# scroll-tech/zkvm-prover

Measured on AMD Instinct MI355X. Metric: chunk STARK proofs/sec (2^22-row trace), higher is better.
Workload: dtype u32; 1 GPU; full STARK proof: 2^22 x 300 degree-3 AIR + 2^22 x 2 Fibonacci AIR, blow-up 2, 100 queries, PoW 16+16 (SURVEY.md 8(d) cfg #4); proof_bytes=1128348, resident_key_bytes_per_pipeline=13503716096, inflight_per_gpu=3, parallelism=3 independent proof(s) in flight per GPU (one HIP stream each)

## Files before the change

### include/zkhip.h

```cpp
#ifndef ZKHIP_H
#define ZKHIP_H
#include <stddef.h>
#include <stdint.h>

#ifdef __cplusplus
extern "C" {
#endif

#define ZKHIP_OK 0
#define ZKHIP_ERR_NO_DEVICE (-1)
#define ZKHIP_ERR_HIP (-2)
#define ZKHIP_ERR_INVALID (-3)
#define ZKHIP_ERR_NOMEM (-4)
#define ZKHIP_ERR_SMALL_BUFFER (-5)
#define ZKHIP_ERR_POW_FAILED (-6)
#define ZKHIP_ERR_VERIFY (-7)
#define ZKHIP_ERR_CONSTRAINT (-8)

#define ZKHIP_DIGEST_WORDS 8

typedef struct zkhip_ctx zkhip_ctx;

uint32_t zkhip_version(void);

// ... 455 lines not shown
int zkhip_recursion_air(const zkhip_recursion *r, size_t i, zkhip_air *out);
int zkhip_recursion_witness(zkhip_recursion *r, const uint8_t *const *proofs, const size_t *proof_lens, const uint32_t *const *const *child_pvs,
                            size_t n_present, uint32_t *node_pvs_out);
int zkhip_recursion_witness_uniform(zkhip_recursion *r, const uint8_t *const *proofs, const size_t *proof_lens, const uint32_t *const *const *child_pvs,
                                    const uint32_t *child_prep_commits, const int *child_is_leaf, const uint32_t leaf_commit[8],
                                    const uint32_t internal_commit[8], size_t n_present, uint32_t *node_pvs_out);
int zkhip_recursion_witness_deferral(zkhip_recursion *r, const uint8_t *const *proofs, const size_t *proof_lens, const uint32_t *const *const *child_pvs,
                                     const uint32_t *child_aux, const uint32_t acc_start[8], size_t n_present, uint32_t *node_pvs_out);
size_t zkhip_recursion_n_aux(const zkhip_recursion *r);
int zkhip_recursion_wires(const zkhip_recursion *r, uint32_t *out, size_t cap_words, size_t *n_words);
int zkhip_recursion_tracegen(zkhip_ctx *ctx, zkhip_recursion *r, uint32_t *d_gate_trace, uint32_t *d_p2_trace, uint32_t *d_pv_trace);

typedef struct {
    int host_sponge;
    uint32_t host_sponge_min_words;
    int jit;
    uint32_t jit_min_log_work;
    char jit_cache_dir[256];
    int quot_slices;
    uint32_t grind_sweep_shift;
    uint32_t coop_max_log, coop_inj_max_log;
    uint32_t top_max_log;
    uint32_t commit_parts, side_cus;
    uint32_t witness_threads;
    int pin_witness, parallel_queries;
    int self_check;
    int tree_store_early;
    uint32_t hash_block;
    int coop_fused;
    int rows_in_bulk;
    uint32_t rows_coop_max_log;
    uint32_t ntt_log_lanes;
    uint32_t quot_streams;
} zkhip_config;
int zkhip_tables_canonical(zkhip_ctx *ctx, int on);
int zkhip_jit_prewarm(const zkhip_air *airs, size_t n_airs, unsigned log_blowup, const char *cache_dir, size_t *n_ok);
void zkhip_config_default(zkhip_config *out);
unsigned zkhip_host_cpus(void);
int zkhip_ctx_get_config(zkhip_ctx *ctx, zkhip_config *out);
int zkhip_has_test_kernels(void);
int zkhip_ctx_set_config(zkhip_ctx *ctx, const zkhip_config *cfg);
int zkhip_set_process_config(const zkhip_config *cfg);

int zkhip_profile_enable(zkhip_ctx *ctx, int on);
typedef struct {
    char name[48];
    uint64_t launches;
    double total_ms;
} zkhip_kernel_stat;
int zkhip_profile_read(zkhip_ctx *ctx, zkhip_kernel_stat *out, size_t cap);
int zkhip_profile_reset(zkhip_ctx *ctx);

#ifdef __cplusplus
}
#endif
#endif
```

### integration/hip-backend/src/ffi.rs

```rust
#![allow(non_camel_case_types)]
use std::os::raw::{c_char, c_double, c_int, c_uint, c_void};

pub const ZKHIP_OK: c_int = 0;
pub const ZKHIP_ERR_NO_DEVICE: c_int = -1;
pub const ZKHIP_ERR_HIP: c_int = -2;
pub const ZKHIP_ERR_INVALID: c_int = -3;
pub const ZKHIP_ERR_NOMEM: c_int = -4;
pub const ZKHIP_ERR_SMALL_BUFFER: c_int = -5;
pub const ZKHIP_ERR_POW_FAILED: c_int = -6;
pub const ZKHIP_ERR_VERIFY: c_int = -7;
pub const ZKHIP_ERR_CONSTRAINT: c_int = -8;
pub const ZKHIP_DIGEST_WORDS: usize = 8;
pub const ZKHIP_KECCAK_F_WIDTH: usize = 2633;
pub const ZKHIP_INT256_ALU_WIDTH: usize = 101;
pub const ZKHIP_INT256_MUL_WIDTH: usize = 161;
pub const ZKHIP_MODMUL_WIDTH: usize = 325;
pub const ZKHIP_EC_WIDTH: usize = 772;
pub const ZKHIP_FP2_WIDTH: usize = 648;
pub const ZKHIP_FP2_RECORD_WORDS: usize = 33;
pub const ZKHIP_INT256_CMP_WIDTH: usize = 103;
pub const ZKHIP_INT256_SHIFT_WIDTH: usize = 189;
pub const ZKHIP_EC_RECORD_WORDS: usize = 41;
pub const ZKHIP_GKR_MAX_LOG_N: c_uint = 28;
pub const ZKHIP_WHIR_MAX_ROUNDS: usize = 32;
// ... 158 lines not shown
    pub uniform: c_int,
    pub min_log_height: [c_uint; 2],
    pub n_leaf_shapes: usize,
    pub app_id: *const u32,
    pub region_index: u32,
}

#[repr(C)]
#[derive(Clone, Copy)]
pub struct zkhip_config {
    pub host_sponge: c_int,
    pub host_sponge_min_words: u32,
    pub jit: c_int,
    pub jit_min_log_work: u32,
    pub jit_cache_dir: [c_char; 256],
    pub quot_slices: c_int,
    pub grind_sweep_shift: u32,
    pub coop_max_log: u32,
    pub coop_inj_max_log: u32,
    pub top_max_log: u32,
    pub commit_parts: u32,
    pub side_cus: u32,
    pub witness_threads: u32,
    pub pin_witness: c_int,
    pub parallel_queries: c_int,
    pub self_check: c_int,
    pub tree_store_early: c_int,
    pub hash_block: u32,
    pub coop_fused: c_int,
    pub rows_in_bulk: c_int,
    pub rows_coop_max_log: u32,
    pub ntt_log_lanes: u32,
    pub quot_streams: u32,
}

#[repr(C)]
#[derive(Clone, Copy)]
pub struct zkhip_kernel_stat {
    pub name: [c_char; 48],
    pub launches: u64,
    pub total_ms: c_double,
}

extern "C" {
    pub fn zkhip_version() -> u32;

    pub fn zkhip_ctx_create(device: c_int, out: *mut *mut zkhip_ctx) -> c_int;
    pub fn zkhip_ctx_destroy(ctx: *mut zkhip_ctx);
    pub fn zkhip_last_error(ctx: *const zkhip_ctx) -> *const c_char;
    pub fn zkhip_set_stream(ctx: *mut zkhip_ctx, hip_stream: *mut c_void) -> c_int;
    pub fn zkhip_sync(ctx: *mut zkhip_ctx) -> c_int;
    pub fn zkhip_set_commit_pipeline(ctx: *mut zkhip_ctx, parts: c_uint) -> c_int;
    pub fn zkhip_set_cu_partition(ctx: *mut zkhip_ctx, side_cus: c_uint) -> c_int;

    pub fn zkhip_malloc(ctx: *mut zkhip_ctx, bytes: usize, dptr: *mut *mut c_void) -> c_int;
    pub fn zkhip_free(ctx: *mut zkhip_ctx, dptr: *mut c_void) -> c_int;
    pub fn zkhip_h2d(ctx: *mut zkhip_ctx, dst: *mut c_void, src: *const c_void, bytes: usize) -> c_int;
    pub fn zkhip_d2h(ctx: *mut zkhip_ctx, dst: *mut c_void, src: *const c_void, bytes: usize) -> c_int;
    pub fn zkhip_host_alloc(ctx: *mut zkhip_ctx, bytes: usize, hptr: *mut *mut c_void) -> c_int;
    pub fn zkhip_host_free(ctx: *mut zkhip_ctx, hptr: *mut c_void) -> c_int;
    pub fn zkhip_h2d_async(ctx: *mut zkhip_ctx, dst: *mut c_void, src_pinned: *const c_void, bytes: usize) -> c_int;
    pub fn zkhip_zero(ctx: *mut zkhip_ctx, dptr: *mut c_void, bytes: usize) -> c_int;
    pub fn zkhip_to_monty(ctx: *mut zkhip_ctx, d: *mut u32, n: usize) -> c_int;
    pub fn zkhip_from_monty(ctx: *mut zkhip_ctx, d: *mut u32, n: usize) -> c_int;

    pub fn zkhip_ntt_batch(ctx: *mut zkhip_ctx, d_mat: *mut u32, log_n: c_uint, width: usize, stride: usize,
// ... 308 lines not shown
```

### zkvm-prover_amd/_binding.py

```python
import ctypes as C
import os
import re

import numpy as np

P = 2013265921
_HERE = os.path.dirname(os.path.abspath(__file__))
_ROOT = os.path.dirname(_HERE)
_LIB = None


class ZkhipError(RuntimeError):
    pass


def library_path():
    return os.path.join(_HERE, "libzkhip.so")


def declared_symbols():
    with open(os.path.join(_ROOT, "include", "zkhip.h")) as f:
        txt = f.read()
    txt = re.sub(r"/\*.*?\*/", "", txt, flags=re.S)
    return sorted(set(re.findall(r"\b(zkhip_[a-z0-9_]+)\s*\(", txt)))
# ... 24 lines not shown
        return p


class _Air(C.Structure):
    _fields_ = [("program", C.POINTER(C.c_uint32)), ("program_len", C.c_size_t), ("log_height", C.c_uint),
                ("width", C.c_size_t), ("n_pvs", C.c_size_t), ("prep_trace", C.POINTER(C.c_uint32)),
                ("prep_commit", C.POINTER(C.c_uint32))]


class _ProofLayout(C.Structure):
    _fields_ = [(n, C.c_size_t) for n in ("n_words", "root_main", "roots_cached", "n_cached", "root_perm", "exposed", "n_exposed", "root_quot", "opened",
                                          "n_opened", "fri_layers", "n_fri_layers", "final_poly", "n_final_poly", "query_pow", "queries",
                                          "query_words", "n_queries")]


class _V1Summary(C.Structure):
    _fields_ = [(n, C.c_size_t) for n in ("n_proofs", "n_airs", "n_queries", "n_fri_layers", "n_final_poly", "n_main_commits",
                                          "n_after_challenge_commits", "n_preprocessed", "n_input_batches")] + \
               [("log_max_height", C.c_uint), ("log_blowup", C.c_uint), ("has_logup_pow", C.c_int), ("log_degree", C.c_uint * 64)]


class _RecursionStmt(C.Structure):
    _fields_ = [("n_state", C.c_size_t), ("start_air", C.POINTER(C.c_uint32)), ("start_idx", C.POINTER(C.c_uint32)),
                ("end_air", C.POINTER(C.c_uint32)), ("end_idx", C.POINTER(C.c_uint32)), ("child_is_node", C.c_int),
                ("uniform", C.c_int), ("min_log_height", C.c_uint * 2), ("n_leaf_shapes", C.c_size_t), ("app_id", C.POINTER(C.c_uint32)),
                ("region_index", C.c_uint32)]


class Config(C.Structure):
    _fields_ = [("host_sponge", C.c_int), ("host_sponge_min_words", C.c_uint32), ("jit", C.c_int), ("jit_min_log_work", C.c_uint32),
                ("jit_cache_dir", C.c_char * 256), ("quot_slices", C.c_int), ("grind_sweep_shift", C.c_uint32), ("coop_max_log", C.c_uint32),
                ("coop_inj_max_log", C.c_uint32), ("top_max_log", C.c_uint32), ("commit_parts", C.c_uint32), ("side_cus", C.c_uint32), ("witness_threads", C.c_uint32),
                ("pin_witness", C.c_int), ("parallel_queries", C.c_int), ("self_check", C.c_int), ("tree_store_early", C.c_int), ("hash_block", C.c_uint32), ("coop_fused", C.c_int),
                ("rows_in_bulk", C.c_int), ("rows_coop_max_log", C.c_uint32), ("ntt_log_lanes", C.c_uint32), ("quot_streams", C.c_uint32)]

    @classmethod
    def default(cls):
        c = cls()
        load_library().zkhip_config_default(C.byref(c))
        return c


class _KernelStat(C.Structure):
    _fields_ = [("name", C.c_char * 48), ("launches", C.c_uint64), ("total_ms", C.c_double)]


def load_library():
    global _LIB
    if _LIB is not None:
        return _LIB
    path = library_path()
    if not os.path.exists(path):
        raise ZkhipError("libzkhip.so not built: run `python -c 'import __graft_entry__ as g; g.build()'` "
                         "(or make -C zkvm-prover_amd/csrc)")
    import torch

    lib = C.CDLL(path)
    vp, sz, u32p, uip = C.c_void_p, C.c_size_t, C.POINTER(C.c_uint32), C.POINTER(C.c_uint)
    sig = {
        "zkhip_version": (C.c_uint32, []),
        "zkhip_ctx_create": (C.c_int, [C.c_int, C.POINTER(vp)]),
        "zkhip_ctx_destroy": (None, [vp]),
        "zkhip_last_error": (C.c_char_p, [vp]),
        "zkhip_set_stream": (C.c_int, [vp, vp]),
        "zkhip_sync": (C.c_int, [vp]),
        "zkhip_set_commit_pipeline": (C.c_int, [vp, C.c_uint]),
        "zkhip_set_cu_partition": (C.c_int, [vp, C.c_uint]),
# ... 1616 lines not shown
```

### zkvm-prover_amd/csrc/api.hip

```cpp
#include <sched.h>
#include <cstring>
#include <thread>
#include <dlfcn.h>
#include <sys/stat.h>
#include <mutex>
#include <string.h>

#include <algorithm>
#include <mutex>
#include <unordered_map>

#include "transcript.hpp"
#include "zkhip_internal.hpp"

namespace zk {

int set_error(zkhip_ctx* ctx, int code, const std::string& msg) {
    if (ctx) ctx->last_error = msg;
    return code;
}

int get_scratch(zkhip_ctx* ctx, int slot, size_t bytes, void** out) {
    if (bytes == 0) bytes = 16;
    if (ctx->scratch_bytes[slot] < bytes) {
// ... 163 lines not shown
    }();
    return cached;
}

void zkhip_config_default(zkhip_config* c) {
    if (!c) return;
    auto num = [](const char* name, uint32_t dflt, uint32_t lo = 0, uint32_t hi = 0xffffffffu) {
        if (!getenv(name)) return dflt;
        const long long v = atoll(getenv(name));
        return (uint32_t)std::min<long long>(hi, std::max<long long>(lo, v));
    };
    memset(c, 0, sizeof *c);
    c->host_sponge = getenv("ZKHIP_NO_HOST_SPONGE") ? 0 : 1;
    c->host_sponge_min_words = num("ZKHIP_HOST_SPONGE_MIN_WORDS", 8192u);
    c->jit = getenv("ZKHIP_NO_JIT") ? 0 : getenv("ZKHIP_FORCE_JIT") ? 2 : 1;
    c->jit_min_log_work = num("ZKHIP_JIT_MIN_LOG_WORK", 26u, 0, 62);
    c->quot_slices = getenv("ZKHIP_NO_QUOT_SLICES") ? 0 : 1;
    c->grind_sweep_shift = num("ZKHIP_GRIND_SWEEP_SHIFT", 0u, 0, 8);
    c->coop_max_log = num("ZKHIP_COOP_MAX_LOG", 15u, 0, 27), c->coop_inj_max_log = num("ZKHIP_COOP_INJ_MAX_LOG", 15u, 0, 27);
    c->top_max_log = num("ZKHIP_TOP_MAX_LOG", 6u, 0, 8);
    c->commit_parts = num("ZKHIP_COMMIT_PARTS", 0u, 0, 8), c->side_cus = num("ZKHIP_SIDE_CUS", 0u);
    c->witness_threads = num("ZKHIP_WITNESS_THREADS", 0u);
    c->pin_witness = getenv("ZKHIP_NO_PIN_WITNESS") ? 0 : 1;
    c->parallel_queries = getenv("ZKHIP_RECURSION_SERIAL_QUERIES") ? 0 : 1;
    c->self_check = getenv("ZKHIP_SELF_CHECK") ? 1 : 0;
#ifdef ZKHIP_TEST_KERNELS
    c->tree_store_early = getenv("ZKHIP_TREE_STORE_EARLY") ? 1 : 0;
#endif
    c->hash_block = num("ZKHIP_HASH_BLOCK", 256u, 64, 768) / 64 * 64;
    c->coop_fused = getenv("ZKHIP_NO_COOP_FUSED") ? 0 : 1;
    c->rows_in_bulk = getenv("ZKHIP_NO_ROWS_IN_BULK") ? 0 : 1;
    c->rows_coop_max_log = num("ZKHIP_ROWS_COOP_MAX_LOG", 15u, 0, 27);
    c->ntt_log_lanes = num("ZKHIP_NTT_LOG_LANES", 10u, 8, 10);
    c->quot_streams = num("ZKHIP_QUOT_STREAMS", 0u, 0, 4);
    std::string dir;
    if (const char* e = getenv("ZKHIP_JIT_CACHE_DIR")) {
        dir = e;
    } else {
        Dl_info info;
        if (dladdr((const void*)&zkhip_config_default, &info) && info.dli_fname) {
            std::string p = info.dli_fname;
            const size_t slash = p.rfind('/');
            p = (slash == std::string::npos ? std::string(".") : p.substr(0, slash)) + "/jit_cache";
            struct stat st;
            if (stat(p.c_str(), &st) == 0 && S_ISDIR(st.st_mode)) dir = p;
        }
    }
    if (dir.size() < sizeof c->jit_cache_dir) memcpy(c->jit_cache_dir, dir.c_str(), dir.size() + 1);
}
extern "C++" {
namespace zk {
static zkhip_config g_process_config;
static std::once_flag g_process_config_once;
static std::mutex g_process_config_mu;
zkhip_config process_config() {
    std::call_once(g_process_config_once, [] { zkhip_config_default(&g_process_config); });
    std::lock_guard<std::mutex> lk(g_process_config_mu);
    return g_process_config;
}
}
}
int zkhip_set_process_config(const zkhip_config* cfg) {
    if (!cfg) return ZKHIP_ERR_INVALID;
    (void)zk::process_config();
    std::lock_guard<std::mutex> lk(zk::g_process_config_mu);
    zk::g_process_config = *cfg;
    return ZKHIP_OK;
}
int zkhip_tables_canonical(zkhip_ctx* ctx, int on) {
    if (!ctx) return ZKHIP_ERR_INVALID;
    ctx->tables_canonical = on != 0;
    return ZKHIP_OK;
}

int zkhip_has_test_kernels(void) {
#ifdef ZKHIP_TEST_KERNELS
    return 1;
#else
    return 0;
#endif
}

int zkhip_ctx_get_config(zkhip_ctx* ctx, zkhip_config* out) {
    if (!ctx || !out) return ZKHIP_ERR_INVALID;
    *out = ctx->cfg;
    return ZKHIP_OK;
}
int zkhip_ctx_set_config(zkhip_ctx* ctx, const zkhip_config* cfg) {
    if (!ctx || !cfg) return ZKHIP_ERR_INVALID;
    if (cfg->jit < 0 || cfg->jit > 2 || cfg->coop_max_log > 27 || cfg->coop_inj_max_log > 27 || cfg->rows_coop_max_log > 27 || cfg->ntt_log_lanes < 8 || cfg->ntt_log_lanes > 10 || cfg->quot_streams > 4 || cfg->jit_min_log_work > 62 || cfg->top_max_log > 8 || cfg->grind_sweep_shift > 8 ||
        cfg->commit_parts > 8 || cfg->side_cus >= (unsigned)ctx->cu_count || cfg->hash_block < 64 || cfg->hash_block > 768 || cfg->hash_block % 64)
        return set_error(ctx, ZKHIP_ERR_INVALID, "zkhip_ctx_set_config: field out of range (jit 0..2, coop_* <= 27, rows_coop_max_log <= 27, ntt_log_lanes 8..10, quot_streams <= 4, jit_min_log_work <= 62, top_max_log <= 8, grind_sweep_shift <= 8, commit_parts <= 8, side_cus < CUs, hash_block a multiple of 64 in 64..768)");
#ifndef ZKHIP_TEST_KERNELS
    if (cfg->tree_store_early)
        return set_error(ctx, ZKHIP_ERR_INVALID, "zkhip_ctx_set_config: tree_store_early names TEST kernels that this library was built without (libzkhip_test.so holds them)");
#endif
    ZK_TRY(zkhip_set_cu_partition(ctx, cfg->side_cus));
    ctx->cfg = *cfg;
    ctx->cfg.jit_cache_dir[sizeof ctx->cfg.jit_cache_dir - 1] = 0;
    ctx->commit_parts = cfg->commit_parts;
    return ZKHIP_OK;
}

void zkhip_ctx_destroy(zkhip_ctx* ctx) {
    if (!ctx) return;
    (void)hipSetDevice(ctx->device);
    (void)hipStreamSynchronize(ctx->stream);
    profile_flush(ctx);
    if (ctx->d_tw_fwd) (void)hipFree(ctx->d_tw_fwd);
    if (ctx->d_tw_inv) (void)hipFree(ctx->d_tw_inv);
    for (auto& kv : ctx->lde_tables) (void)hipFree(kv.second);
    for (int i = 0; i < 8; i++)
        if (ctx->scratch[i]) (void)hipFree(ctx->scratch[i]);
    if (ctx->side_stream) (void)hipStreamDestroy(ctx->side_stream);
    if (ctx->hash_stream) (void)hipStreamDestroy(ctx->hash_stream);
    for (auto& q : ctx->quot_streams)
        if (q) (void)hipStreamDestroy(q);
    if (ctx->quot_fork) (void)hipEventDestroy(ctx->quot_fork);
    for (auto& e : ctx->quot_join)
        if (e) (void)hipEventDestroy(e);
    if (ctx->d_deferred_bad) (void)hipFree(ctx->d_deferred_bad);
    if (ctx->gkr_ws) (void)hipFree(ctx->gkr_ws);
    if (ctx->h_sponge) (void)hipHostFree(ctx->h_sponge);
    if (ctx->own_stream) (void)hipStreamDestroy(ctx->own_stream);
    for (auto& e : ctx->pipe_ev)
// ... 340 lines not shown
```

### zkvm-prover_amd/csrc/ntt.hip

```cpp
#include <stdlib.h>
#include <string.h>

#include <algorithm>

#include "lds_barrier.hpp"
#include "zkhip_internal.hpp"

namespace zk {

__global__ void k_gen_twiddles(uint32_t* fwd, uint32_t* inv, uint32_t w, uint32_t winv, size_t half) {
    size_t e = (size_t)blockIdx.x * blockDim.x + threadIdx.x;
    if (e >= half) return;
    fwd[e] = mpow(w, e);
    inv[e] = mpow(winv, e);
}

int ensure_twiddles(zkhip_ctx* ctx, unsigned log_n) {
    if (log_n < 1) log_n = 1;
    if (log_n > 27) return set_error(ctx, ZKHIP_ERR_INVALID, "transform size exceeds two-adicity 27");
    if (ctx->tw_log >= log_n) return ZKHIP_OK;
    unsigned want = std::max(log_n, 16u);
    if (ctx->d_tw_fwd) {
        ZK_HIP_CHECK(ctx, hipStreamSynchronize(ctx->stream));
        ZK_HIP_CHECK(ctx, hipFree(ctx->d_tw_fwd));
// ... 403 lines not shown
#endif
        uint32_t* base = lv + j * pitch + c;
#pragma unroll
        for (int k = 0; k < 16; k++) base[(k << LOG_RQ) * pitch] = v[k];
    }
    zk_syncthreads();
#if !defined(NTT_ABL) || (NTT_ABL != 4 && NTT_ABL != 5)
    lds_rounds_ct<LOG_R, LOG_C, LOG_RQ, NT>(lv, twl, tid);
#endif
    const unsigned lo_mask = (1u << a.log_lo) - 1u;
    uint32_t* dst = (a.dst_cols ? a.dst_cols[mcol] : a.dst + mcol * a.dst_col_stride) + ((size_t)sub << a.log_m) + (size_t)X * a.out_x_stride;
    if constexpr (LOG_R >= LOG_T) {
        const uint32_t* lrow = lv + tid * pitch;
#pragma unroll
        for (unsigned i = 0; i < (R * C) / NT; i++) {
            const unsigned c = (NT * i) >> LOG_R, p0 = (NT * i) & (R - 1u);
            const unsigned F = F0 + c;
            uint32_t* dcol = dst + (size_t)(F >> a.log_lo) * a.out_hi_stride + (size_t)(F & lo_mask) * a.out_lo_stride + p0;
#if defined(NTT_ABL) && NTT_ABL == 3
            if (lrow[p0 * pitch + c] == 0x12345678u) dcol[tid] = 1;
#else
            dcol[tid] = lrow[p0 * pitch + c];
#endif
        }
    } else {
        const unsigned p = tid & (R - 1u), c_lane = tid >> LOG_R;
        const uint32_t* lrow = lv + p * pitch + c_lane;
#pragma unroll
        for (unsigned i = 0; i < (R * C) / NT; i++) {
            const unsigned F = F0 + c_lane + i * (NT >> LOG_R);
            uint32_t* dcol = dst + (size_t)(F >> a.log_lo) * a.out_hi_stride + (size_t)(F & lo_mask) * a.out_lo_stride + p;
            *dcol = lrow[i * (NT >> LOG_R)];
        }
    }
}

struct LdeFusedArgs {
    const uint32_t* src;
    size_t src_col_stride;
    uint32_t* dst;
    size_t dst_col_stride;
    const uint32_t *tw_inv, *tw_fwd;
    unsigned tw_log, log_m, log_cosets;
    const uint32_t *scale_col, *scale_row, *scale_rho;
};
template <int LOG_R, int LOG_C, int MIN_WAVES>
__global__ __launch_bounds__(1024, MIN_WAVES) void k_ntt_lde_fused(LdeFusedArgs a) {
    constexpr int LOG_T = 10;
    static_assert(LOG_R - 4 + LOG_C == LOG_T, "one radix-16 unit per lane");
    constexpr unsigned NT = 1u << LOG_T;
    extern __shared__ uint32_t sm[];
    constexpr unsigned R = 1u << LOG_R, C = 1u << LOG_C, pitch = C + 1u;
    constexpr int LOG_RQ = LOG_R - 4;
    constexpr unsigned log_f = LOG_R;
    uint32_t* lv = sm;
    uint32_t* twl = sm + R * pitch;
    const unsigned tid = threadIdx.x;
    for (unsigned e = tid; e < (R >> 1); e += NT) twl[e] = a.tw_inv[(size_t)e << (a.tw_log - LOG_R)];
    const size_t mcol = blockIdx.y;
    unsigned tile = blockIdx.x;
    if (LOG_C == 3) {
        unsigned k = gridDim.x >> 3;
        if (k > 16u) k = 16u;
        if (k >= 2u && (k & (k - 1u)) == 0 && (gridDim.x & (8u * k - 1u)) == 0) {
            const unsigned within = tile & (8u * k - 1u);
            tile = (tile & ~(8u * k - 1u)) | ((within & 7u) * k) | (within >> 3);
// ... 93 lines not shown
    if (!v) {
        const char* e = getenv("ZKHIP_NTT_MAX_LOG_R");
        v = e ? (unsigned)atoi(e) : P4_MAX_LOG_R;
        if (v < 9 || v > P4_MAX_LOG_R) v = P4_MAX_LOG_R;
    }
    return v;
}

struct BrSrc {
    const uint32_t *scale_col, *scale_row, *scale_rho;
};
static unsigned fourstep_split(unsigned log_n, unsigned a[3]) {
    const unsigned n_pass = std::max(2u, (log_n + p4_log_r_limit() - 1) / p4_log_r_limit());
    a[0] = a[1] = a[2] = 0;
    for (unsigned p = 0; p < n_pass; p++) a[p] = log_n / n_pass + (p < log_n % n_pass ? 1 : 0);
    return n_pass;
}

static int ntt_dif_fourstep(zkhip_ctx* ctx, const uint32_t* src, size_t src_stride, uint32_t* dst, size_t dst_stride,
                            uint32_t* tmp, uint32_t* tmp2, size_t tmp_stride, unsigned log_n, size_t width,
                            unsigned log_sub, bool inverse, const BrSrc* brsrc = nullptr,
                            const uint32_t* const* src_cols = nullptr, uint32_t* const* dst_cols = nullptr) {
    static DeviceOnce attr_set;
    if (attr_set.need(ctx->device)) {
        const int lds_max = ((17u << P4_MAX_LOG_R) + (1u << (P4_MAX_LOG_R - 1))) * 4;
        ZK_HIP_CHECK(ctx, hipFuncSetAttribute((const void*)k_ntt_pass4<11, 3>, hipFuncAttributeMaxDynamicSharedMemorySize, lds_max));
        ZK_HIP_CHECK(ctx, hipFuncSetAttribute((const void*)k_ntt_pass4<10, 4>, hipFuncAttributeMaxDynamicSharedMemorySize, lds_max));
        ZK_HIP_CHECK(ctx, hipFuncSetAttribute((const void*)k_ntt_pass4_ct<11, 3>, hipFuncAttributeMaxDynamicSharedMemorySize, lds_max));
        ZK_HIP_CHECK(ctx, hipFuncSetAttribute((const void*)k_ntt_pass4_ct<10, 4>, hipFuncAttributeMaxDynamicSharedMemorySize, lds_max));
        ZK_HIP_CHECK(ctx, hipFuncSetAttribute((const void*)k_ntt_pass4_ct<9, 5>, hipFuncAttributeMaxDynamicSharedMemorySize, lds_max));
        ZK_HIP_CHECK(ctx, hipFuncSetAttribute((const void*)k_ntt_pass4_ct<8, 6>, hipFuncAttributeMaxDynamicSharedMemorySize, lds_max));
        ZK_HIP_CHECK(ctx, hipFuncSetAttribute((const void*)k_ntt_pass4_ct<7, 7>, hipFuncAttributeMaxDynamicSharedMemorySize, lds_max));
        ZK_HIP_CHECK(ctx, hipFuncSetAttribute((const void*)k_ntt_pass4<0, 0>, hipFuncAttributeMaxDynamicSharedMemorySize, lds_max));
        attr_set.mark(ctx->device);
    }
    unsigned a[3];
    const unsigned n_pass = fourstep_split(log_n, a);
    const uint32_t* tw = inverse ? ctx->d_tw_inv : ctx->d_tw_fwd;
    auto launch = [&](Pass4Args& pa, const uint32_t* s, size_t ss, uint32_t* d, size_t ds, unsigned n_x) -> int {
        pa.src = s;
        pa.src_col_stride = ss;
        pa.dst = d;
        pa.dst_col_stride = ds;
        pa.tw = tw;
        pa.tw_log = ctx->tw_log;
        pa.log_sub = log_sub;
        pa.log_m = log_n;
        const unsigned R = 1u << pa.log_r;
        static int log_c_env = -1;
        if (log_c_env < 0) {
            const char* e = getenv("ZKHIP_NTT_LOG_C");
            log_c_env = e ? atoi(e) : 0;
            if (log_c_env != 3 && log_c_env != 4) log_c_env = 0;
        }
        pa.log_c = log_c_env ? (unsigned)log_c_env : (pa.log_r >= 11 ? 3u : (pa.log_r >= 7 ? 14u - pa.log_r : 4u));
        unsigned log_t = 10;
        if (!log_c_env && pa.log_r >= 7 && pa.log_r <= 10 && ctx->cfg.ntt_log_lanes >= 8 && ctx->cfg.ntt_log_lanes <= 9) {
            const unsigned lc = ctx->cfg.ntt_log_lanes + 4 - pa.log_r;
            if (lc >= 2 && lc <= pa.log_f) log_t = ctx->cfg.ntt_log_lanes, pa.log_c = lc;
        }
        if (pa.log_c > pa.log_f) pa.log_c = pa.log_f;
        const unsigned C = 1u << pa.log_c;
        const unsigned threads = std::min(1024u, std::max(64u, (R >> 4) * C));
        const size_t lds = ((size_t)R * (C + 1) + (R >> 1)) * 4;
        dim3 grid(n_x << (pa.log_f - pa.log_c), (unsigned)(width << log_sub));
        KernelScope ks(ctx, inverse ? "ntt_pass_inv" : "ntt_pass_fwd");
        static const bool legacy = getenv("ZKHIP_NTT_LEGACY") != nullptr;
        static const unsigned prio_env = getenv("ZKHIP_NTT_PRIO") ? (unsigned)atoi(getenv("ZKHIP_NTT_PRIO")) : 0u;
        pa.prio = prio_env;
#define ZK_NTT_CT(R_, C_, T_) hipLaunchKernelGGL((k_ntt_pass4_ct<R_, C_, T_>), grid, dim3(1u << T_), lds, ctx->stream, pa)
        if (log_t == 9 && pa.log_r == 10 && pa.log_c == 3) ZK_NTT_CT(10, 3, 9);
        else if (log_t == 9 && pa.log_r == 9 && pa.log_c == 4) ZK_NTT_CT(9, 4, 9);
        else if (log_t == 9 && pa.log_r == 8 && pa.log_c == 5) ZK_NTT_CT(8, 5, 9);
        else if (log_t == 9 && pa.log_r == 7 && pa.log_c == 6) ZK_NTT_CT(7, 6, 9);
        else if (log_t == 8 && pa.log_r == 10 && pa.log_c == 2) ZK_NTT_CT(10, 2, 8);
        else if (log_t == 8 && pa.log_r == 9 && pa.log_c == 3) ZK_NTT_CT(9, 3, 8);
        else if (log_t == 8 && pa.log_r == 8 && pa.log_c == 4) ZK_NTT_CT(8, 4, 8);
        else if (log_t == 8 && pa.log_r == 7 && pa.log_c == 5) ZK_NTT_CT(7, 5, 8);
#undef ZK_NTT_CT
        else if (pa.log_r == 11 && pa.log_c == 3 && !legacy)
            hipLaunchKernelGGL((k_ntt_pass4_ct<11, 3>), grid, dim3(threads), lds, ctx->stream, pa);
        else if (pa.log_r == 10 && pa.log_c == 4 && !legacy)
            hipLaunchKernelGGL((k_ntt_pass4_ct<10, 4>), grid, dim3(threads), lds, ctx->stream, pa);
        else if (pa.log_r == 9 && pa.log_c == 5 && !legacy)
            hipLaunchKernelGGL((k_ntt_pass4_ct<9, 5>), grid, dim3(threads), lds, ctx->stream, pa);
        else if (pa.log_r == 8 && pa.log_c == 6 && !legacy)
            hipLaunchKernelGGL((k_ntt_pass4_ct<8, 6>), grid, dim3(threads), lds, ctx->stream, pa);
        else if (pa.log_r == 7 && pa.log_c == 7 && !legacy)
            hipLaunchKernelGGL((k_ntt_pass4_ct<7, 7>), grid, dim3(threads), lds, ctx->stream, pa);
        else if (pa.log_r == 11 && pa.log_c == 3)
            hipLaunchKernelGGL((k_ntt_pass4<11, 3>), grid, dim3(threads), lds, ctx->stream, pa);
        else if (pa.log_r == 10 && pa.log_c == 4)
            hipLaunchKernelGGL((k_ntt_pass4<10, 4>), grid, dim3(threads), lds, ctx->stream, pa);
        else
            hipLaunchKernelGGL((k_ntt_pass4<0, 0>), grid, dim3(threads), lds, ctx->stream, pa);
        ZK_HIP_CHECK(ctx, hipGetLastError());
        return ZKHIP_OK;
    };
    Pass4Args pa;
    memset(&pa, 0, sizeof pa);
    auto first_pass_src = [&]() {
        if (brsrc) {
            pa.br_src = 1;
            pa.scale_col = brsrc->scale_col, pa.scale_row = brsrc->scale_row, pa.scale_rho = brsrc->scale_rho;
        }
    };
    if (n_pass == 2) {
        const unsigned a1 = a[0], a2 = a[1];
        pa.log_r = a1, pa.log_f = a2, pa.in_x_stride = 0, pa.in_rs = (size_t)1 << a2;
        pa.out_x_stride = 0, pa.out_hi_stride = (size_t)1 << a1, pa.out_lo_stride = 0, pa.log_lo = 0, pa.in_tw = 0;
        first_pass_src();
        pa.src_cols = src_cols;
        ZK_TRY(launch(pa, src, src_stride, tmp, tmp_stride, 1));
// ... 6 lines not shown
        pa.src_cols = nullptr, pa.dst_cols = nullptr;
    } else {
        const unsigned a1 = a[0], a2 = a[1], a3 = a[2];
        pa.log_r = a1, pa.log_f = a2 + a3, pa.in_x_stride = 0, pa.in_rs = (size_t)1 << (a2 + a3);
        pa.out_x_stride = 0, pa.log_lo = a3, pa.out_lo_stride = (size_t)1 << (a1 + a2), pa.out_hi_stride = (size_t)1 << a1;
        pa.in_tw = 0;
        first_pass_src();
        pa.src_cols = src_cols;
        ZK_TRY(launch(pa, src, src_stride, tmp, tmp_stride, 1));
        pa.src_cols = nullptr, pa.dst_cols = nullptr;
        pa.br_src = 0;
        pa.log_r = a2, pa.log_f = a1, pa.in_x_stride = (size_t)1 << (a1 + a2), pa.in_rs = (size_t)1 << a1;
        pa.out_x_stride = (size_t)1 << a2, pa.log_lo = 0, pa.out_lo_stride = 0, pa.out_hi_stride = (size_t)1 << (a2 + a3);
        pa.in_tw = 1, pa.log_prev = a1, pa.log_tt = log_n, pa.tw_a = 1u << a3, pa.tw_bx = 1;
        ZK_TRY(launch(pa, tmp, tmp_stride, tmp2, tmp_stride, 1u << a3));
        pa.log_r = a3, pa.log_f = a2, pa.in_x_stride = (size_t)1 << (a2 + a3), pa.in_rs = (size_t)1 << a2;
        pa.out_x_stride = (size_t)1 << (a2 + a3), pa.out_hi_stride = (size_t)1 << a3;
        pa.in_tw = 1, pa.log_prev = a2, pa.log_tt = a2 + a3, pa.tw_a = 1, pa.tw_bx = 0;
        pa.dst_cols = dst_cols;
        ZK_TRY(launch(pa, tmp2, tmp_stride, dst, dst_stride, 1u << a1));
        pa.src_cols = nullptr, pa.dst_cols = nullptr;
    }
    return ZKHIP_OK;
}

static constexpr unsigned MAX_LOG_R = 11;
static constexpr unsigned MAX_LOG_TILE = 15;
static constexpr unsigned MAX_LOG_C = 7;

int ntt_dif_inplace(zkhip_ctx* ctx, const uint32_t* src, size_t src_stride, uint32_t* dst, size_t dst_stride,
                    unsigned log_n, size_t width, unsigned log_sub, bool inverse) {
    if (width == 0) return ZKHIP_OK;
    ZK_TRY(ensure_twiddles(ctx, log_n));
    if (log_n >= P4_MIN_LOG_M) {
        const size_t per_col = (size_t)1 << (log_n + log_sub);
        const bool three = log_n > 2 * p4_log_r_limit();
        void* tmp;
        ZK_TRY(get_scratch(ctx, 4, per_col * width * 4 * (three ? 2 : 1), &tmp));
        uint32_t* t1 = (uint32_t*)tmp;
        uint32_t* t2 = three ? t1 + per_col * width : nullptr;
        return ntt_dif_fourstep(ctx, src, src_stride, dst, dst_stride, t1, t2, per_col, log_n, width, log_sub, inverse);
    }
    if (log_n == 0) {
        if (src != dst) {
            ZK_HIP_CHECK(ctx, hipMemcpy2DAsync(dst, dst_stride * 4, src, src_stride * 4, 4u << log_sub, width,
                                               hipMemcpyDeviceToDevice, ctx->stream));
        }
        return ZKHIP_OK;
    }
    static DeviceOnce attr_set;
    if (attr_set.need(ctx->device)) {
        ZK_HIP_CHECK(ctx, hipFuncSetAttribute((const void*)k_ntt_dif_pass,
                                              hipFuncAttributeMaxDynamicSharedMemorySize, 4 << MAX_LOG_TILE));
        attr_set.mark(ctx->device);
    }
    unsigned n_pass = (log_n + MAX_LOG_R - 1) / MAX_LOG_R;
    unsigned base = log_n / n_pass, rem = log_n % n_pass;
    unsigned s0 = 0;
    for (unsigned p = 0; p < n_pass; p++) {
        PassArgs a;
        a.src = (p == 0) ? src : dst;
        a.src_stride = (p == 0) ? src_stride : dst_stride;
        a.dst = dst;
        a.dst_stride = dst_stride;
        a.tw = inverse ? ctx->d_tw_inv : ctx->d_tw_fwd;
        a.log_m = log_n;
        a.s0 = s0;
// ... 283 lines not shown
        fa.scale_col = d_col, fa.scale_row = d_row, fa.scale_rho = d_rho;
        KernelScope ks(ctx, "ntt_lde_fused");
        const dim3 grid(1u << (a1 - 3), (unsigned)width);
        const bool one_wg = getenv("ZKHIP_LDE_FUSED_WAVES") && atoi(getenv("ZKHIP_LDE_FUSED_WAVES")) == 4;
        if (one_wg) hipLaunchKernelGGL((k_ntt_lde_fused<11, 3, 4>), grid, dim3(1024), (size_t)lds, ctx->stream, fa);
        else hipLaunchKernelGGL((k_ntt_lde_fused<11, 3, 8>), grid, dim3(1024), (size_t)lds, ctx->stream, fa);
        ZK_HIP_CHECK(ctx, hipGetLastError());
    }
    {
        Pass4Args pa;
        memset(&pa, 0, sizeof pa);
        pa.log_r = a2, pa.log_f = a1, pa.in_x_stride = 0, pa.in_rs = (size_t)1 << a1;
        pa.out_x_stride = 0, pa.out_hi_stride = (size_t)1 << a2, pa.out_lo_stride = 0, pa.log_lo = 0;
        pa.in_tw = 1, pa.log_prev = a1, pa.log_tt = log_n, pa.tw_a = 1, pa.tw_bx = 0;
        pa.src = t2, pa.src_col_stride = per_col;
        pa.dst = d_out, pa.dst_col_stride = out_stride, pa.dst_cols = d_dst_cols;
        pa.tw = ctx->d_tw_fwd, pa.tw_log = ctx->tw_log, pa.log_sub = added_bits, pa.log_m = log_n, pa.log_c = 3;
        KernelScope ks(ctx, "ntt_pass_fwd");
        const dim3 grid(1u << (pa.log_f - pa.log_c), (unsigned)(width << added_bits));
        const size_t lds2 = ((((size_t)1 << a2) * 9u) + ((size_t)1 << (a2 - 1))) * 4;
        hipLaunchKernelGGL((k_ntt_pass4_ct<11, 3>), grid, dim3(1024), lds2, ctx->stream, pa);
        ZK_HIP_CHECK(ctx, hipGetLastError());
    }
    return ZKHIP_OK;
}

int lde_batch(zkhip_ctx* ctx, const uint32_t* d_in, size_t in_stride, uint32_t* d_out, size_t out_stride,
              unsigned log_n, unsigned added_bits, size_t width, uint32_t shift_monty) {
    if (width == 0) return ZKHIP_OK;
    const size_t n = (size_t)1 << log_n;
    if (in_stride < n || out_stride < (n << added_bits)) return set_error(ctx, ZKHIP_ERR_INVALID, "stride < height");
    if (log_n + added_bits > 27) return set_error(ctx, ZKHIP_ERR_INVALID, "LDE size exceeds two-adicity");
    ZK_TRY(ensure_twiddles(ctx, log_n + added_bits));
    if (lde_fused_applies(log_n)) return lde_fused(ctx, d_in, in_stride, nullptr, d_out, out_stride, nullptr, log_n, added_bits, width, shift_monty);
    void* coeffs;
    ZK_TRY(get_scratch(ctx, 0, n * width * 4, &coeffs));
    ZK_TRY(ntt_dif_inplace(ctx, d_in, in_stride, (uint32_t*)coeffs, n, log_n, width, 0, true));
    if (log_n >= P4_MIN_LOG_M) {
        unsigned a[3];
        fourstep_split(log_n, a);
        const unsigned log_f = log_n - a[0], log_rq = a[0] - 4, n_co = 1u << added_bits;
        const size_t n_col = (size_t)1 << log_f, n_row = (size_t)1 << log_rq;
        uint32_t* d_col = nullptr;
        ZK_TRY(lde_scale_tables(ctx, log_n, added_bits, shift_monty, log_f, log_rq, &d_col));
        uint32_t* d_row = d_col + n_co * n_col;
        uint32_t* d_rho = d_row + n_co * n_row;
        BrSrc bs{d_col, d_row, d_rho};
        const size_t per_col = n << added_bits;
        const bool three = log_n > 2 * p4_log_r_limit();
        void* tmp;
        ZK_TRY(get_scratch(ctx, 4, per_col * width * 4 * (three ? 2 : 1), &tmp));
        uint32_t* t1 = (uint32_t*)tmp;
        uint32_t* t2 = three ? t1 + per_col * width : nullptr;
        return ntt_dif_fourstep(ctx, (const uint32_t*)coeffs, n, d_out, out_stride, t1, t2, per_col, log_n, width, added_bits,
                                false, &bs);
    }
    unsigned lb = (log_n + 1) / 2;
    unsigned per = (1u << lb) + (1u << (log_n - lb));
    uint32_t* pw = nullptr;
    {
        const uint64_t key = ((uint64_t)1 << 63) | ((uint64_t)log_n << 56) | ((uint64_t)added_bits << 48) | shift_monty;
        auto it = ctx->lde_tables.find(key);
        if (it == ctx->lde_tables.end()) {
            const unsigned cnt = per << added_bits, bs = 256;
            if (hipMalloc(&pw, (size_t)cnt * 4) != hipSuccess) return set_error(ctx, ZKHIP_ERR_NOMEM, "lde power tables");
            {
                KernelScope ks(ctx, "gen_coset_powers");
                const uint32_t n_inv = minv(to_monty((uint32_t)(n % P)));
                hipLaunchKernelGGL(k_gen_coset_powers, dim3((cnt + bs - 1) / bs), dim3(bs), 0, ctx->stream, pw, shift_monty, two_adic_generator(log_n + added_bits), n_inv, log_n,
                                   added_bits, lb);
            }
// ... 70 lines not shown
```

Before: 12.60 proofs/s.

## Add specialized square 2^11x2^11 four-step NTT pass kernel for 2^22 transforms

Adds a specialized Cooley-Tukey four-step pass kernel for the square 2^22 case (2^11 x 8 tiles, 1024 lanes). It has compile-time modes for plain, inline-twiddle geometric scaling and bit-reversed-source LDE scaling, with wave-uniform base pointers via readfirstlane and a swizzled tile order. With the default form 0 it replaces the generic k_ntt_pass4_ct<11,3> for matching launches, aiming to cut address arithmetic and improve memory access locality. A new config knob also allows falling back to non-fourstep paths (form 2), which adds branching and risks divergence from the generic path's coverage conditions.

```diff
diff --git a/include/zkhip.h b/include/zkhip.h
--- a/include/zkhip.h
+++ b/include/zkhip.h
@@ -511,6 +511,7 @@
     uint32_t rows_coop_max_log;
     uint32_t ntt_log_lanes;
     uint32_t quot_streams;
+    uint32_t ntt_pass_form;
 } zkhip_config;
 int zkhip_tables_canonical(zkhip_ctx *ctx, int on);
 int zkhip_jit_prewarm(const zkhip_air *airs, size_t n_airs, unsigned log_blowup, const char *cache_dir, size_t *n_ok);
diff --git a/integration/hip-backend/src/ffi.rs b/integration/hip-backend/src/ffi.rs
--- a/integration/hip-backend/src/ffi.rs
+++ b/integration/hip-backend/src/ffi.rs
@@ -214,6 +214,7 @@
     pub rows_coop_max_log: u32,
     pub ntt_log_lanes: u32,
     pub quot_streams: u32,
+    pub ntt_pass_form: u32,
 }
 
 #[repr(C)]
diff --git a/zkvm-prover_amd/_binding.py b/zkvm-prover_amd/_binding.py
--- a/zkvm-prover_amd/_binding.py
+++ b/zkvm-prover_amd/_binding.py
@@ -80,7 +80,7 @@
                 ("jit_cache_dir", C.c_char * 256), ("quot_slices", C.c_int), ("grind_sweep_shift", C.c_uint32), ("coop_max_log", C.c_uint32),
                 ("coop_inj_max_log", C.c_uint32), ("top_max_log", C.c_uint32), ("commit_parts", C.c_uint32), ("side_cus", C.c_uint32), ("witness_threads", C.c_uint32),
                 ("pin_witness", C.c_int), ("parallel_queries", C.c_int), ("self_check", C.c_int), ("tree_store_early", C.c_int), ("hash_block", C.c_uint32), ("coop_fused", C.c_int),
-                ("rows_in_bulk", C.c_int), ("rows_coop_max_log", C.c_uint32), ("ntt_log_lanes", C.c_uint32), ("quot_streams", C.c_uint32)]
+                ("rows_in_bulk", C.c_int), ("rows_coop_max_log", C.c_uint32), ("ntt_log_lanes", C.c_uint32), ("quot_streams", C.c_uint32), ("ntt_pass_form", C.c_uint32)]
 
     @classmethod
     def default(cls):
diff --git a/zkvm-prover_amd/csrc/api.hip b/zkvm-prover_amd/csrc/api.hip
--- a/zkvm-prover_amd/csrc/api.hip
+++ b/zkvm-prover_amd/csrc/api.hip
@@ -219,6 +219,7 @@
     c->rows_in_bulk = getenv("ZKHIP_NO_ROWS_IN_BULK") ? 0 : 1;
     c->rows_coop_max_log = num("ZKHIP_ROWS_COOP_MAX_LOG", 15u, 0, 27);
     c->ntt_log_lanes = num("ZKHIP_NTT_LOG_LANES", 10u, 8, 10);
+    c->ntt_pass_form = num("ZKHIP_NTT_PASS_FORM", 0u, 0, 2);
     c->quot_streams = num("ZKHIP_QUOT_STREAMS", 0u, 0, 4);
     std::string dir;
     if (const char* e = getenv("ZKHIP_JIT_CACHE_DIR")) {
@@ -275,9 +276,9 @@
 }
 int zkhip_ctx_set_config(zkhip_ctx* ctx, const zkhip_config* cfg) {
     if (!ctx || !cfg) return ZKHIP_ERR_INVALID;
-    if (cfg->jit < 0 || cfg->jit > 2 || cfg->coop_max_log > 27 || cfg->coop_inj_max_log > 27 || cfg->rows_coop_max_log > 27 || cfg->ntt_log_lanes < 8 || cfg->ntt_log_lanes > 10 || cfg->quot_streams > 4 || cfg->jit_min_log_work > 62 || cfg->top_max_log > 8 || cfg->grind_sweep_shift > 8 ||
+    if (cfg->jit < 0 || cfg->jit > 2 || cfg->coop_max_log > 27 || cfg->coop_inj_max_log > 27 || cfg->rows_coop_max_log > 27 || cfg->ntt_log_lanes < 8 || cfg->ntt_log_lanes > 10 || cfg->ntt_pass_form > 2 || cfg->quot_streams > 4 || cfg->jit_min_log_work > 62 || cfg->top_max_log > 8 || cfg->grind_sweep_shift > 8 ||
         cfg->commit_parts > 8 || cfg->side_cus >= (unsigned)ctx->cu_count || cfg->hash_block < 64 || cfg->hash_block > 768 || cfg->hash_block % 64)
-        return set_error(ctx, ZKHIP_ERR_INVALID, "zkhip_ctx_set_config: field out of range (jit 0..2, coop_* <= 27, rows_coop_max_log <= 27, ntt_log_lanes 8..10, quot_streams <= 4, jit_min_log_work <= 62, top_max_log <= 8, grind_sweep_shift <= 8, commit_parts <= 8, side_cus < CUs, hash_block a multiple of 64 in 64..768)");
+        return set_error(ctx, ZKHIP_ERR_INVALID, "zkhip_ctx_set_config: field out of range (jit 0..2, coop_* <= 27, rows_coop_max_log <= 27, ntt_log_lanes 8..10, ntt_pass_form <= 2, quot_streams <= 4, jit_min_log_work <= 62, top_max_log <= 8, grind_sweep_shift <= 8, commit_parts <= 8, side_cus < CUs, hash_block a multiple of 64 in 64..768)");
 #ifndef ZKHIP_TEST_KERNELS
     if (cfg->tree_store_early)
         return set_error(ctx, ZKHIP_ERR_INVALID, "zkhip_ctx_set_config: tree_store_early names TEST kernels that this library was built without (libzkhip_test.so holds them)");
diff --git a/zkvm-prover_amd/csrc/ntt.hip b/zkvm-prover_amd/csrc/ntt.hip
--- a/zkvm-prover_amd/csrc/ntt.hip
+++ b/zkvm-prover_amd/csrc/ntt.hip
@@ -459,6 +459,103 @@
             uint32_t* dcol = dst + (size_t)(F >> a.log_lo) * a.out_hi_stride + (size_t)(F & lo_mask) * a.out_lo_stride + p;
             *dcol = lrow[i * (NT >> LOG_R)];
         }
+    }
+}
+
+struct ShapeSq11 {
+    static constexpr int LOG_R = 11, LOG_C = 3, LOG_T = 10;
+};
+enum : int { P4_PLAIN = 0, P4_IN_TW = 1, P4_BR_SRC = 2 };
+
+__device__ __forceinline__ void scale_geometric(uint32_t (&v)[16], uint32_t t, uint32_t rho) {
+    int32_t ts = (int32_t)t;
+    v[0] = canon_signed(smml((int32_t)v[0], ts));
+#pragma unroll
+    for (int k = 1; k < 16; k++) {
+        ts = smml(ts, (int32_t)rho);
+        v[k] = canon_signed(smml((int32_t)v[k], ts));
+    }
+}
+
+typedef __attribute__((address_space(1))) uint32_t* global_words;
+__device__ __forceinline__ global_words uniform_global(const uint32_t* p) {
+    const uint64_t x = (uint64_t)p;
+    const uint32_t lo = __builtin_amdgcn_readfirstlane((uint32_t)x), hi = __builtin_amdgcn_readfirstlane((uint32_t)(x >> 32));
+    return (global_words)(((uint64_t)hi << 32) | lo);
+}
+__device__ __forceinline__ global_words uniform_global(global_words p) {
+    const uint64_t x = (uint64_t)p;
+    const uint32_t lo = __builtin_amdgcn_readfirstlane((uint32_t)x), hi = __builtin_amdgcn_readfirstlane((uint32_t)(x >> 32));
+    return (global_words)(((uint64_t)hi << 32) | lo);
+}
+
+template <class SH, int MODE>
+__global__ __launch_bounds__(1 << SH::LOG_T, 8) void k_ntt_pass4_ct_sq(Pass4Args a) {
+    constexpr int LOG_R = SH::LOG_R, LOG_C = SH::LOG_C, LOG_T = SH::LOG_T;
+    constexpr int LOG_F = LOG_R, LOG_M = 2 * LOG_R, LOG_RQ = LOG_R - 4;
+    constexpr unsigned NT = 1u << LOG_T, R = 1u << LOG_R, C = 1u << LOG_C, pitch = C + 1u;
+    static_assert(LOG_C == 3 && LOG_RQ + LOG_C == LOG_T && LOG_R >= LOG_T && (R >> 1) % NT == 0 && LOG_F - LOG_C >= 7, "[2^11 x 8] tiles of 1024 lanes");
+    if (a.prio == 3) __builtin_amdgcn_s_setprio(3);
+    else if (a.prio == 2) __builtin_amdgcn_s_setprio(2);
+    else if (a.prio == 1) __builtin_amdgcn_s_setprio(1);
+    extern __shared__ uint32_t sm[];
+    uint32_t* lv = sm;
+    uint32_t* twl = sm + R * pitch;
+    const unsigned tid = threadIdx.x;
+    const unsigned col = blockIdx.y;
+    const unsigned sub = col & ((1u << a.log_sub) - 1u);
+    const size_t mcol = col >> a.log_sub;
+    unsigned tile = blockIdx.x;
+    tile = (tile & ~127u) | ((tile & 7u) << 4) | ((tile & 127u) >> 3);
+    const unsigned F0 = tile << LOG_C;
+    const unsigned c = tid & (C - 1u), jj = tid >> LOG_C;
+    const unsigned j = ((jj & 3u) << 3) | ((jj >> 2) & 7u) | (jj & ~31u);
+    uint32_t twe[(R >> 1) / NT];
+#pragma unroll
+    for (unsigned i = 0; i < (R >> 1) / NT; i++) twe[i] = a.tw[(size_t)(tid + i * NT) << (a.tw_log - LOG_R)];
+    uint32_t t = 0, rho = 0, v[16];
+    if constexpr (MODE == P4_BR_SRC) {
+        const uint32_t sc = a.scale_col[((size_t)sub << LOG_F) + F0 + c], sr = a.scale_row[((size_t)sub << LOG_RQ) + j];
+        rho = a.scale_rho[sub];
+        const uint32_t* run = a.src + mcol * a.src_col_stride + ((size_t)bitrev32(F0 + c, LOG_F) << LOG_R);
+        const uint4* ch = reinterpret_cast<const uint4*>(run + ((size_t)bitrev32(j, LOG_RQ) << 4));
+        const uint4 q0 = ch[0], q1 = ch[1], q2 = ch[2], q3 = ch[3];
+        const uint32_t wv[16] = {q0.x, q0.y, q0.z, q0.w, q1.x, q1.y, q1.z, q1.w, q2.x, q2.y, q2.z, q2.w, q3.x, q3.y, q3.z, q3.w};
+#pragma unroll
+        for (int k = 0; k < 16; k++) v[k] = wv[((k & 1) << 3) | ((k & 2) << 1) | ((k & 4) >> 1) | ((k & 8) >> 3)];
+        t = mmul(sc, sr);
+    } else {
+        if constexpr (MODE == P4_IN_TW) {
+            const uint32_t kc = bitrev32(F0 + c, LOG_F);
+            const unsigned sh = a.tw_log - LOG_M;
+            t = a.tw[(size_t)(kc * j) << sh];
+            rho = a.tw[(size_t)(kc << LOG_RQ) << sh];
+        }
+        const global_words tile_src = uniform_global((a.src_cols ? a.src_cols[mcol] : a.src + mcol * a.src_col_stride) + ((size_t)sub << LOG_M) + F0);
+        const uint32_t lane_off = (j << LOG_F) + c;
+#pragma unroll
+        for (int k = 0; k < 16; k++) v[k] = uniform_global(tile_src + ((size_t)k << (LOG_RQ + LOG_F)))[lane_off];
+    }
+#pragma unroll
+    for (unsigned i = 0; i < (R >> 1) / NT; i++) twl[tid + i * NT] = twe[i];
+    if constexpr (MODE != P4_PLAIN) scale_geometric(v, t, rho);
+    zk_syncthreads();
+    {
+        uint32_t w[15];
+        load_unit_twiddles<4, LOG_RQ, 0>(twl, j, w);
+        dif_unit_w<4>(v, w);
+        uint32_t* base = lv + j * pitch + c;
+#pragma unroll
+        for (int k = 0; k < 16; k++) base[(k << LOG_RQ) * pitch] = v[k];
+    }
+    zk_syncthreads();
+    lds_rounds_ct<LOG_R, LOG_C, LOG_RQ, NT>(lv, twl, tid);
+    const global_words dst = uniform_global((a.dst_cols ? a.dst_cols[mcol] : a.dst + mcol * a.dst_col_stride) + ((size_t)sub << LOG_M) + ((size_t)F0 << LOG_R));
+    const uint32_t* lrow = lv + tid * pitch;
+#pragma unroll
+    for (unsigned i = 0; i < (R * C) / NT; i++) {
+        const unsigned cc = (NT * i) >> LOG_R, p0 = (NT * i) & (R - 1u);
+        uniform_global(dst + ((size_t)cc << LOG_R) + p0)[tid] = lrow[p0 * pitch + cc];
     }
 }
 
@@ -618,6 +715,9 @@
         ZK_HIP_CHECK(ctx, hipFuncSetAttribute((const void*)k_ntt_pass4_ct<8, 6>, hipFuncAttributeMaxDynamicSharedMemorySize, lds_max));
         ZK_HIP_CHECK(ctx, hipFuncSetAttribute((const void*)k_ntt_pass4_ct<7, 7>, hipFuncAttributeMaxDynamicSharedMemorySize, lds_max));
         ZK_HIP_CHECK(ctx, hipFuncSetAttribute((const void*)k_ntt_pass4<0, 0>, hipFuncAttributeMaxDynamicSharedMemorySize, lds_max));
+        ZK_HIP_CHECK(ctx, hipFuncSetAttribute((const void*)k_ntt_pass4_ct_sq<ShapeSq11, P4_PLAIN>, hipFuncAttributeMaxDynamicSharedMemorySize, lds_max));
+        ZK_HIP_CHECK(ctx, hipFuncSetAttribute((const void*)k_ntt_pass4_ct_sq<ShapeSq11, P4_IN_TW>, hipFuncAttributeMaxDynamicSharedMemorySize, lds_max));
+        ZK_HIP_CHECK(ctx, hipFuncSetAttribute((const void*)k_ntt_pass4_ct_sq<ShapeSq11, P4_BR_SRC>, hipFuncAttributeMaxDynamicSharedMemorySize, lds_max));
         attr_set.mark(ctx->device);
     }
     unsigned a[3];
@@ -664,7 +764,13 @@
         else if (log_t == 8 && pa.log_r == 8 && pa.log_c == 4) ZK_NTT_CT(8, 4, 8);
         else if (log_t == 8 && pa.log_r == 7 && pa.log_c == 5) ZK_NTT_CT(7, 5, 8);
 #undef ZK_NTT_CT
-        else if (pa.log_r == 11 && pa.log_c == 3 && !legacy)
+        else if (ctx->cfg.ntt_pass_form == 0 && !legacy && n_pass == 2 && n_x == 1 && log_n == 22 && pa.log_r == 11 && pa.log_f == 11 && pa.log_c == 3 &&
+                 pa.log_lo == 0 && pa.in_x_stride == 0 && pa.out_x_stride == 0 && pa.out_hi_stride == ((size_t)1 << 11) && !(pa.br_src && pa.in_tw) &&
+                 (!pa.in_tw || (pa.log_prev == 11 && pa.log_tt == 22 && pa.tw_a == 1 && pa.tw_bx == 0))) {
+            if (pa.br_src) hipLaunchKernelGGL((k_ntt_pass4_ct_sq<ShapeSq11, P4_BR_SRC>), grid, dim3(1024), lds, ctx->stream, pa);
+            else if (pa.in_tw) hipLaunchKernelGGL((k_ntt_pass4_ct_sq<ShapeSq11, P4_IN_TW>), grid, dim3(1024), lds, ctx->stream, pa);
+            else hipLaunchKernelGGL((k_ntt_pass4_ct_sq<ShapeSq11, P4_PLAIN>), grid, dim3(1024), lds, ctx->stream, pa);
+        } else if (pa.log_r == 11 && pa.log_c == 3 && !legacy)
             hipLaunchKernelGGL((k_ntt_pass4_ct<11, 3>), grid, dim3(threads), lds, ctx->stream, pa);
         else if (pa.log_r == 10 && pa.log_c == 4 && !legacy)
             hipLaunchKernelGGL((k_ntt_pass4_ct<10, 4>), grid, dim3(threads), lds, ctx->stream, pa);
@@ -737,7 +843,7 @@
                     unsigned log_n, size_t width, unsigned log_sub, bool inverse) {
     if (width == 0) return ZKHIP_OK;
     ZK_TRY(ensure_twiddles(ctx, log_n));
-    if (log_n >= P4_MIN_LOG_M) {
+    if (log_n >= P4_MIN_LOG_M && ctx->cfg.ntt_pass_form != 2) {
         const size_t per_col = (size_t)1 << (log_n + log_sub);
         const bool three = log_n > 2 * p4_log_r_limit();
         void* tmp;
@@ -1087,11 +1193,11 @@
     if (in_stride < n || out_stride < (n << added_bits)) return set_error(ctx, ZKHIP_ERR_INVALID, "stride < height");
     if (log_n + added_bits > 27) return set_error(ctx, ZKHIP_ERR_INVALID, "LDE size exceeds two-adicity");
     ZK_TRY(ensure_twiddles(ctx, log_n + added_bits));
-    if (lde_fused_applies(log_n)) return lde_fused(ctx, d_in, in_stride, nullptr, d_out, out_stride, nullptr, log_n, added_bits, width, shift_monty);
+    if (lde_fused_applies(log_n) && ctx->cfg.ntt_pass_form != 2) return lde_fused(ctx, d_in, in_stride, nullptr, d_out, out_stride, nullptr, log_n, added_bits, width, shift_monty);
     void* coeffs;
     ZK_TRY(get_scratch(ctx, 0, n * width * 4, &coeffs));
     ZK_TRY(ntt_dif_inplace(ctx, d_in, in_stride, (uint32_t*)coeffs, n, log_n, width, 0, true));
-    if (log_n >= P4_MIN_LOG_M) {
+    if (log_n >= P4_MIN_LOG_M && ctx->cfg.ntt_pass_form != 2) {
         unsigned a[3];
         fourstep_split(log_n, a);
         const unsigned log_f = log_n - a[0], log_rq = a[0] - 4, n_co = 1u << added_bits;
```

New measurement: 12.78 proofs/s, median of 6. +1.5%, better.
